# VinAIResearch/Counting-DETR

Measured on AMD Instinct MI355X. Metric: images/sec FSCD-147 2nd-stage train step, higher is better.
Workload: dtype forward bf16x3 (fp32 operands split hi+lo, 3 bf16 MFMAs per product); data / weight gradients bf16 (both operands rounded to bf16, 1 MFMA per product); fp32 accumulate, fp32 storage, fp32 attention softmax / norms / losses / optimizer; 1 GPU; FSCD-147 2nd-stage train step (ResNet-50-DC5 + RCDA enc6/dec6, Q=300 learned, 800x800, T=[37, 120]), fwd+matcher+loss+bwd+clip+AdamW; images_per_gpu=2, global_batch=2, parallelism=dp1, graph=True, precision=bf16x3, precision_backward=bf16, frozen_stage_prefetch=True

## Files before the change

### counting_detr_amd/csrc/api.hip

```cpp
#include <stdarg.h>
#include <stdio.h>

#include "../../include/cdetr_hip.h"
#include "common.h"

static thread_local char g_err[512] = "";

void cdetr_set_error(const char* fmt, ...) {
    va_list ap;
    va_start(ap, fmt);
    vsnprintf(g_err, sizeof(g_err), fmt, ap);
    va_end(ap);
}

extern "C" const char* cdetr_last_error(void) { return g_err; }
extern "C" int cdetr_abi_version(void) { return CDETR_ABI_VERSION; }

#include <stdlib.h>
#include <string.h>
extern char** environ;
namespace {
struct TuneEnvCheck {
    TuneEnvCheck() {
        if (getenv("CDETR_TUNING") != nullptr || environ == nullptr) return;
        static const char* const knobs[] = {"CDETR_DIRECT_MAX_BLOCKS", "CDETR_GEMM_DL", "CDETR_GEMM_FEWROW_SPLIT", "CDETR_GEMM_SPLITK", "CDETR_GEMM_VARIANT",
                                            "CDETR_LN_BWD_ROWS", "CDETR_LSAP_GENERIC", "CDETR_RCDA_HS", "CDETR_RCDA_PROBE", "CDETR_WGRAD_KP",
                                            "CDETR_WGRAD_VARIANT"};
        for (const char* k : knobs)
            if (getenv(k) != nullptr)
                fprintf(stderr, "libcdetr_hip: %s is set but CDETR_TUNING is not -- per-call tuning knobs are ignored without it\n", k);
    }
} g_tune_env_check;
}
```

### counting_detr_amd/csrc/matcher.hip

```cpp
#include "../../include/cdetr_hip.h"
#include "common.h"
#include <stdlib.h>

#pragma clang fp contract(off)

namespace {

__global__ __launch_bounds__(256) void match_cost_kernel(const float* __restrict__ logits, int ncls,
                                                         const float* __restrict__ boxes, const float* __restrict__ tgt,
                                                         const int* __restrict__ tgt_off, const int64_t* __restrict__ cost_off,
                                                         int Q, float w_class, float w_bbox, float w_giou,
                                                         float* __restrict__ cost) {
    const int b = blockIdx.y;
    const int t0 = tgt_off[b], T = tgt_off[b + 1] - t0;
    const long total = (long)Q * T;
    const bool transpose = T < Q;
    float* out = cost + cost_off[b];
    for (long idx = (long)blockIdx.x * 256 + threadIdx.x; idx < total; idx += (long)gridDim.x * 256) {
        int q, t;
        if (transpose) { t = (int)(idx / Q); q = (int)(idx - (long)t * Q); }
        else { q = (int)(idx / T); t = (int)(idx - (long)q * T); }
        const float x = logits[((long)b * Q + q) * ncls + 0];
        const float p = 1.f / (1.f + expf(-x));
        const float neg = (0.75f * (p * p)) * (-logf((1.f - p) + 1e-8f));
        const float pos = (0.25f * ((1.f - p) * (1.f - p))) * (-logf(p + 1e-8f));
        const float cost_class = pos - neg;
        const float* ob = boxes + ((long)b * Q + q) * 4;
        const float* tb = tgt + ((long)t0 + t) * 4;
        const float ocx = ob[0], ocy = ob[1], ow = ob[2], oh = ob[3];
        const float tcx = tb[0], tcy = tb[1], tw = tb[2], th = tb[3];
        const float cost_bbox = ((fabsf(ocx - tcx) + fabsf(ocy - tcy)) + fabsf(ow - tw)) + fabsf(oh - th);
        const float ox0 = ocx - 0.5f * ow, oy0 = ocy - 0.5f * oh, ox1 = ocx + 0.5f * ow, oy1 = ocy + 0.5f * oh;
        const float tx0 = tcx - 0.5f * tw, ty0 = tcy - 0.5f * th, tx1 = tcx + 0.5f * tw, ty1 = tcy + 0.5f * th;
        const float a1 = (ox1 - ox0) * (oy1 - oy0), a2 = (tx1 - tx0) * (ty1 - ty0);
        const float iw = fmaxf(fminf(ox1, tx1) - fmaxf(ox0, tx0), 0.f), ih = fmaxf(fminf(oy1, ty1) - fmaxf(oy0, ty0), 0.f);
        const float inter = iw * ih;
        const float uni = (a1 + a2) - inter;
        const float iou = inter / uni;
        const float ew = fmaxf(fmaxf(ox1, tx1) - fminf(ox0, tx0), 0.f), eh = fmaxf(fmaxf(oy1, ty1) - fminf(oy0, ty0), 0.f);
        const float area = ew * eh;
        const float giou = iou - (area - uni) / area;
        const float c = (w_bbox * cost_bbox + w_class * cost_class) + w_giou * (-giou);
        out[idx] = c;
    }
}

struct Cand {
    double val;
    int it;
    int unassigned;
};
__device__ __forceinline__ Cand better(const Cand& a, const Cand& b) {
    if (a.it < 0) return b;
    if (b.it < 0) return a;
    if (a.val < b.val) return a;
    if (b.val < a.val) return b;
    if (a.unassigned != b.unassigned) return a.unassigned ? a : b;
    if (a.unassigned) return (a.it > b.it) ? a : b;
    return (a.it < b.it) ? a : b;
}
__device__ __forceinline__ Cand shfl_xor_cand(const Cand& c, int m) {
    Cand r;
    r.val = __shfl_xor(c.val, m, 64);
    r.it = __shfl_xor(c.it, m, 64);
    r.unassigned = __shfl_xor(c.unassigned, m, 64);
    return r;
}

template <int NT>
__global__ __launch_bounds__(NT) void lsap_kernel(const float* __restrict__ cost_all, const int64_t* __restrict__ cost_off,
                                                  const int* __restrict__ tgt_off, int Q, int Mmax, int64_t* __restrict__ idx_i,
                                                  int64_t* __restrict__ idx_j, int* __restrict__ status, int nc_cap) {
    extern __shared__ __attribute__((aligned(16))) unsigned char lds[];
    __builtin_amdgcn_s_setprio(3);
    const int b = blockIdx.x;
    const int T = tgt_off[b + 1] - tgt_off[b];
    const bool transpose = T < Q;
    const int nr = transpose ? T : Q;
    const int nc = transpose ? Q : T;
    const float* cost = cost_all + cost_off[b];
    const int tid = threadIdx.x;
    int64_t* oi = idx_i + (long)b * Mmax;
    int64_t* oj = idx_j + (long)b * Mmax;
    for (int i = tid; i < Mmax; i += NT) { oi[i] = 0; oj[i] = 0; }
    __syncthreads();
    if (nr == 0) { if (tid == 0) status[b] = 0; return; }

    double* v = reinterpret_cast<double*>(lds);
    double* spc = v + nc_cap;
    double* u = spc + nc_cap;
    int* path = reinterpret_cast<int*>(u + nc_cap);
    int* row4col = path + nc_cap;
    int* remaining = row4col + nc_cap;
    int* col4row = remaining + nc_cap;
    unsigned char* SC = reinterpret_cast<unsigned char*>(col4row + nc_cap);
    unsigned char* SR = SC + nc_cap;
    __shared__ Cand wave_best[NT / 64];
    __shared__ int s_i, s_sink, s_num_remaining, s_bad;
    __shared__ double s_min;

    if (tid == 0) s_bad = 0;
    for (int j = tid; j < nc; j += NT) { v[j] = 0.0; path[j] = -1; row4col[j] = -1; }
    for (int i = tid; i < nr; i += NT) { u[i] = 0.0; col4row[i] = -1; }
    __syncthreads();
    {
        int bad = 0;
        for (long k = tid; k < (long)nr * nc; k += NT) {
            const float c = cost[k];
            if (c != c || c == -INFINITY) bad = 1;
        }
        if (bad) atomicOr(&s_bad, 1);
    }
    __syncthreads();
    if (s_bad) { if (tid == 0) status[b] = 2; return; }

    for (int cur = 0; cur < nr; ++cur) {
        for (int j = tid; j < nc; j += NT) { spc[j] = INFINITY; SC[j] = 0; remaining[j] = nc - j - 1; }
        for (int i = tid; i < nr; i += NT) SR[i] = 0;
        if (tid == 0) { s_i = cur; s_sink = -1; s_num_remaining = nc; s_min = 0.0; }
        __syncthreads();
        while (true) {
            const int i = s_i;
            const int num_remaining = s_num_remaining;
            const double min_val = s_min;
            const double ui = u[i];
            const float* crow = cost + (long)i * nc;
            Cand best;
            best.val = INFINITY; best.it = -1; best.unassigned = 0;
            for (int it = tid; it < num_remaining; it += NT) {
                const int j = remaining[it];
                const double r = ((min_val + (double)crow[j]) - ui) - v[j];
                double s = spc[j];
                if (r < s) { path[j] = i; spc[j] = r; s = r; }
                Cand c;
                c.val = s; c.it = it; c.unassigned = (row4col[j] == -1);
                best = better(best, c);
            }
#pragma unroll
            for (int m = 32; m > 0; m >>= 1) best = better(best, shfl_xor_cand(best, m));
            if (NT > 64) {
                if ((tid & 63) == 0) wave_best[tid >> 6] = best;
                __syncthreads();
                if (tid == 0) {
                    Cand bb = wave_best[0];
                    for (int wv = 1; wv < NT / 64; ++wv) bb = better(bb, wave_best[wv]);
                    wave_best[0] = bb;
                }
                __syncthreads();
                best = wave_best[0];
            }
            if (tid == 0) {
                SR[i] = 1;
                if (best.it < 0 || best.val == INFINITY) {
                    s_sink = -2;
                } else {
                    const int j = remaining[best.it];
                    s_min = best.val;
                    if (row4col[j] == -1) s_sink = j;
                    else s_i = row4col[j];
                    SC[j] = 1;
                    remaining[best.it] = remaining[num_remaining - 1];
                    s_num_remaining = num_remaining - 1;
                }
            }
            __syncthreads();
            if (s_sink != -1) break;
        }
        const int sink = s_sink;
        if (sink == -2) { if (tid == 0) status[b] = 1; return; }
        const double min_val = s_min;
        for (int i = tid; i < nr; i += NT) {
            if (i == cur) u[i] += min_val;
            else if (SR[i]) u[i] += min_val - spc[col4row[i]];
        }
        for (int j = tid; j < nc; j += NT)
            if (SC[j]) v[j] -= min_val - spc[j];
        __syncthreads();
        if (tid == 0) {
            int j = sink;
            while (true) {
                const int i = path[j];
                row4col[j] = i;
                const int t = col4row[i];
                col4row[i] = j;
                j = t;
                if (i == cur) break;
            }
        }
        __syncthreads();
    }
    if (!transpose) {
        for (int i = tid; i < nr; i += NT) { oi[i] = i; oj[i] = col4row[i]; }
    } else {
        for (int j = tid; j < nc; j += NT) remaining[j] = (row4col[j] != -1) ? 1 : 0;
        __syncthreads();
        if (tid == 0) {
            int run = 0;
            for (int j = 0; j < nc; ++j) { const int f = remaining[j]; remaining[j] = run; run += f; }
        }
        __syncthreads();
        for (int j = tid; j < nc; j += NT)
            if (row4col[j] != -1) { oi[remaining[j]] = j; oj[remaining[j]] = row4col[j]; }
    }
    if (tid == 0) status[b] = 0;
}


template <int CTRL, int ROW_MASK>
__device__ __forceinline__ double dpp_min_f64(double x) {
    const int lo = __double2loint(x), hi = __double2hiint(x);
    const int olo = __builtin_amdgcn_update_dpp(lo, lo, CTRL, ROW_MASK, 0xf, false);
    const int ohi = __builtin_amdgcn_update_dpp(hi, hi, CTRL, ROW_MASK, 0xf, false);
    const double o = __hiloint2double(ohi, olo);
    return (o < x) ? o : x;
}
template <int CTRL, int ROW_MASK>
__device__ __forceinline__ unsigned dpp_min_u32(unsigned x) {
    const unsigned o = (unsigned)__builtin_amdgcn_update_dpp((int)x, (int)x, CTRL, ROW_MASK, 0xf, false);
    return o < x ? o : x;
}
__device__ __forceinline__ void wave_lexmin(double& val, unsigned& key) {
    double m = val;
    m = dpp_min_f64<0xB1, 0xf>(m);
    m = dpp_min_f64<0x4E, 0xf>(m);
    m = dpp_min_f64<0x141, 0xf>(m);
    m = dpp_min_f64<0x140, 0xf>(m);
    m = dpp_min_f64<0x142, 0xa>(m);
    m = dpp_min_f64<0x143, 0xc>(m);
    const double gmin = __hiloint2double(__builtin_amdgcn_readlane(__double2hiint(m), 63), __builtin_amdgcn_readlane(__double2loint(m), 63));
    unsigned k = (val == gmin) ? key : 0xffffffffu;
    k = dpp_min_u32<0xB1, 0xf>(k);
    k = dpp_min_u32<0x4E, 0xf>(k);
    k = dpp_min_u32<0x141, 0xf>(k);
    k = dpp_min_u32<0x140, 0xf>(k);
    k = dpp_min_u32<0x142, 0xa>(k);
    k = dpp_min_u32<0x143, 0xc>(k);
    key = (unsigned)__builtin_amdgcn_readlane((int)k, 63);
    val = gmin;
}

template <int CPL, bool COST_LDS>
__global__ __launch_bounds__(64) void lsap_wave_kernel(const float* __restrict__ cost_all, const int64_t* __restrict__ cost_off,
                                                       const int* __restrict__ tgt_off, int Q, int Mmax,
                                                       int64_t* __restrict__ idx_i, int64_t* __restrict__ idx_j,
                                                       int* __restrict__ status) {
    extern __shared__ __attribute__((aligned(16))) unsigned char lds[];
    __builtin_amdgcn_s_setprio(3);
    const int b = blockIdx.x;
    const int T = tgt_off[b + 1] - tgt_off[b];
    const bool transpose = T < Q;
    const int nr = transpose ? T : Q;
    const int nc = transpose ? Q : T;
    const float* cost_g = cost_all + cost_off[b];
    const int lane = threadIdx.x;
    int64_t* oi = idx_i + (long)b * Mmax;
    int64_t* oj = idx_j + (long)b * Mmax;
    for (int i = lane; i < Mmax; i += 64) { oi[i] = 0; oj[i] = 0; }
    if (nr == 0) { if (lane == 0) status[b] = 0; return; }

    double* u = reinterpret_cast<double*>(lds);
    int* col4row = reinterpret_cast<int*>(u + nr);
    int* row4col = col4row + nr;
    int* remaining = row4col + nc;
    int* pathl = remaining + nc;
    float* cost_l = reinterpret_cast<float*>((reinterpret_cast<uintptr_t>(pathl + nc) + 15) & ~(uintptr_t)15);
    const float* cost = COST_LDS ? cost_l : cost_g;

    int bad = 0;
    const long ntot = (long)nr * nc;
    constexpr int LU = 16;
    if ((reinterpret_cast<uintptr_t>(cost_g) & 15) == 0) {
        const long n4 = ntot >> 2;
        const float4* g4 = reinterpret_cast<const float4*>(cost_g);
        for (long k0 = 0; k0 < n4; k0 += 64 * LU) {
            float4 t[LU];
#pragma unroll
            for (int q = 0; q < LU; ++q) t[q] = g4[min(k0 + lane + 64 * q, n4 - 1)];
#pragma unroll
            for (int q = 0; q < LU; ++q) {
                const long k = k0 + lane + 64 * q;
                if (k < n4) {
                    const float4 c = t[q];
                    if (c.x != c.x || c.x == -INFINITY || c.y != c.y || c.y == -INFINITY || c.z != c.z || c.z == -INFINITY ||
                        c.w != c.w || c.w == -INFINITY) bad = 1;
                    if (COST_LDS) *reinterpret_cast<float4*>(cost_l + 4 * k) = c;
                }
            }
        }
        for (long k = (n4 << 2) + lane; k < ntot; k += 64) {
            const float c = cost_g[k];
            if (c != c || c == -INFINITY) bad = 1;
            if (COST_LDS) cost_l[k] = c;
        }
    } else {
        for (long k0 = 0; k0 < ntot; k0 += 64 * LU) {
            float t[LU];
#pragma unroll
            for (int q = 0; q < LU; ++q) t[q] = cost_g[min(k0 + lane + 64 * q, ntot - 1)];
#pragma unroll
            for (int q = 0; q < LU; ++q) {
                const long k = k0 + lane + 64 * q;
                if (k < ntot) {
                    if (t[q] != t[q] || t[q] == -INFINITY) bad = 1;
                    if (COST_LDS) cost_l[k] = t[q];
                }
            }
        }
    }
    if (__any(bad)) { if (lane == 0) status[b] = 2; return; }
    for (int i = lane; i < nr; i += 64) { u[i] = 0.0; col4row[i] = -1; }
    for (int j = lane; j < nc; j += 64) row4col[j] = -1;

    double v[CPL], spc[CPL];
    int path[CPL], r4c[CPL];
    unsigned key[CPL];
    unsigned valid = 0;
#pragma unroll
    for (int c = 0; c < CPL; ++c) { v[c] = 0.0; path[c] = -1; r4c[c] = -1; if (lane + 64 * c < nc) valid |= 1u << c; }

    for (int cur = 0; cur < nr; ++cur) {
        {
            const float* crow0 = cost + (long)cur * nc;
            const double ui0 = u[cur];
            const double min0 = 0.0;
            double bval = INFINITY;
            unsigned bkey = 0xffffffffu;
            int best_c = 0;
#pragma unroll
            for (int c = 0; c < CPL; ++c) {
                const bool a = (valid >> c) & 1u;
                const int jj = a ? lane + 64 * c : 0;
                const double r = ((min0 + (double)crow0[jj]) - ui0) - v[c];
                const double s = (a & (r < INFINITY)) ? r : INFINITY;
                const unsigned p0 = (unsigned)(nc - 1 - (lane + 64 * c));
                const unsigned k = (r4c[c] == -1) ? (0x7fffffffu - p0) : (0x80000000u + p0);
                const bool better = a & ((s < bval) | ((s == bval) & (k < bkey)));
                bval = better ? s : bval;
                bkey = better ? k : bkey;
                best_c = better ? c : best_c;
            }
            const double my_val = bval;
            const unsigned my_key = bkey;
            wave_lexmin(bval, bkey);
            if (bkey != 0xffffffffu && bval != INFINITY && (bkey & 0x80000000u) == 0u) {
                const bool mine = (my_key == bkey) && (my_val == bval);
                const int wl = __builtin_ctzll(__ballot(mine));
                const int jstar = __builtin_amdgcn_readlane(lane + 64 * best_c, wl);
                if (lane == 0) {
                    u[cur] = ui0 + bval;
                    row4col[jstar] = cur;
                    col4row[cur] = jstar;
                }
#pragma unroll
                for (int c = 0; c < CPL; ++c) r4c[c] = (mine && best_c == c) ? cur : r4c[c];
                continue;
            }
        }
        unsigned sc = 0;
#pragma unroll
        for (int c = 0; c < CPL; ++c) {
            spc[c] = INFINITY;
            const unsigned p0 = (unsigned)(nc - 1 - (lane + 64 * c));
            key[c] = (r4c[c] == -1) ? (0x7fffffffu - p0) : (0x80000000u + p0);
        }
        for (int it = lane; it < nc; it += 64) remaining[it] = nc - 1 - it;
        int i = cur, num_remaining = nc, sink = -1;
        double min_val = 0.0;
        while (true) {
            const int last = num_remaining - 1;
            const int jlast = *reinterpret_cast<volatile int*>(remaining + last);
            const float* crow = cost + (long)i * nc;
            const double ui = u[i];
            double bval = INFINITY;
            unsigned bkey = 0xffffffffu;
            int best_c = 0;
            const unsigned act = valid & ~sc;
#pragma unroll
            for (int c = 0; c < CPL; ++c) {
                const bool a = (act >> c) & 1u;
                const int jj = ((valid >> c) & 1u) ? lane + 64 * c : 0;
                const double r = ((min_val + (double)crow[jj]) - ui) - v[c];
                const bool upd = a & (r < spc[c]);
                spc[c] = upd ? r : spc[c];
                path[c] = upd ? i : path[c];
                const bool better = a & ((spc[c] < bval) | ((spc[c] == bval) & (key[c] < bkey)));
                bval = better ? spc[c] : bval;
                bkey = better ? key[c] : bkey;
                best_c = better ? c : best_c;
            }
            const double my_val = bval;
            const unsigned my_key = bkey;
            wave_lexmin(bval, bkey);
            if (bkey == 0xffffffffu || bval == INFINITY) { sink = -2; break; }
            min_val = bval;
            const bool mine = (my_key == bkey) && (my_val == bval);
            const int wl = __builtin_ctzll(__ballot(mine));
            int my_r = r4c[0];
#pragma unroll
            for (int c = 1; c < CPL; ++c) my_r = (best_c == c) ? r4c[c] : my_r;
            const int jstar = __builtin_amdgcn_readlane(lane + 64 * best_c, wl);
            const int inext = __builtin_amdgcn_readlane(my_r, wl);
            const bool j_unassigned = (bkey & 0x80000000u) == 0u;
            const int best_it = j_unassigned ? (int)(0x7fffffffu - bkey) : (int)(bkey - 0x80000000u);
            sc |= mine ? (1u << best_c) : 0u;
            if (lane == 0) remaining[best_it] = jlast;
#pragma unroll
            for (int c = 0; c < CPL; ++c) {
                const unsigned nk = (r4c[c] == -1) ? (0x7fffffffu - (unsigned)best_it) : (0x80000000u + (unsigned)best_it);
                key[c] = (lane + 64 * c == jlast) ? nk : key[c];
            }
            num_remaining = last;
            if (j_unassigned) { sink = jstar; break; }
            i = inext;
        }
        if (sink == -2) { if (lane == 0) status[b] = 1; return; }
        if (lane == 0) u[cur] += min_val;
#pragma unroll
        for (int c = 0; c < CPL; ++c) {
            const int j = lane + 64 * c;
            if ((sc >> c) & 1u) {
                const double delta = min_val - spc[c];
                v[c] -= delta;
                if (j != sink) u[r4c[c]] += delta;
            }
            if (j < nc) pathl[j] = path[c];
        }
        if (lane == 0) {
            int j = sink;
            while (true) {
                const int ii = pathl[j];
                row4col[j] = ii;
                const int t = col4row[ii];
                col4row[ii] = j;
                j = t;
                if (ii == cur) break;
            }
        }
#pragma unroll
        for (int c = 0; c < CPL; ++c)
            if ((valid >> c) & 1u) r4c[c] = row4col[lane + 64 * c];
    }
    if (!transpose) {
        for (int i = lane; i < nr; i += 64) { oi[i] = i; oj[i] = col4row[i]; }
    } else {
        int base = 0;
        for (int j0 = 0; j0 < nc; j0 += 64) {
            const int j = j0 + lane;
            const int r = (j < nc) ? row4col[j] : -1;
            const unsigned long long m = __ballot(r != -1);
            if (r != -1) {
                const int rank = base + __popcll(m & ((1ull << lane) - 1ull));
                oi[rank] = j;
                oj[rank] = r;
            }
            base += __popcll(m);
        }
    }
    if (lane == 0) status[b] = 0;
}

struct WgSlot { double val; unsigned key; int jstar; int rnext; int pad_; };

template <int CPL>
__global__ __launch_bounds__(1024) void lsap_wg_kernel(const float* __restrict__ cost_all, const int64_t* __restrict__ cost_off,
                                                       const int* __restrict__ tgt_off, int Q, int Mmax, int64_t* __restrict__ idx_i,
                                                       int64_t* __restrict__ idx_j, int* __restrict__ status) {
    constexpr int NT = 1024, NW = 16;
    extern __shared__ __attribute__((aligned(16))) unsigned char lds[];
    __builtin_amdgcn_s_setprio(3);
    const int b = blockIdx.x;
    const int T = tgt_off[b + 1] - tgt_off[b];
    const bool transpose = T < Q;
    const int nr = transpose ? T : Q;
    const int nc = transpose ? Q : T;
    const float* __restrict__ cost = cost_all + cost_off[b];
    const int tid = threadIdx.x, lane = tid & 63, wv = tid >> 6;
    int64_t* oi = idx_i + (long)b * Mmax;
    int64_t* oj = idx_j + (long)b * Mmax;
    for (int i = tid; i < Mmax; i += NT) { oi[i] = 0; oj[i] = 0; }
    if (nr == 0) { if (tid == 0) status[b] = 0; return; }

    WgSlot* slots = reinterpret_cast<WgSlot*>(lds);
    double* u = reinterpret_cast<double*>(slots + 2 * NW);
    int* col4row = reinterpret_cast<int*>(u + nr);
    int* row4col = col4row + nr;
    int* remaining = row4col + nc;
    int* pathl = remaining + nc;
    __shared__ int s_bad;
    if (tid == 0) s_bad = 0;
    for (int i = tid; i < nr; i += NT) { u[i] = 0.0; col4row[i] = -1; }
    for (int j = tid; j < nc; j += NT) row4col[j] = -1;
    __syncthreads();
    {
        int bad = 0;
        const long ntot = (long)nr * nc;
        for (long k0 = 0; k0 < ntot; k0 += (long)NT * 8) {
            float t[8];
#pragma unroll
            for (int q = 0; q < 8; ++q) t[q] = cost[min(k0 + tid + (long)NT * q, ntot - 1)];
#pragma unroll
            for (int q = 0; q < 8; ++q) bad |= (t[q] != t[q] || t[q] == -INFINITY) ? 1 : 0;
        }
        if (bad) atomicOr(&s_bad, 1);
    }
    __syncthreads();
    if (s_bad) { if (tid == 0) status[b] = 2; return; }

    double v[CPL], spc[CPL];
    int path[CPL], r4c[CPL];
    unsigned key[CPL];
    unsigned valid = 0;
#pragma unroll
    for (int c = 0; c < CPL; ++c) { v[c] = 0.0; spc[c] = INFINITY; path[c] = -1; r4c[c] = -1; key[c] = 0xffffffffu; if (tid + NT * c < nc) valid |= 1u << c; }
    int parity = 0;

    auto wg_lexmin = [&](double& bval, unsigned& bkey, int best_c, int& jstar, int& rnext, bool& mine) __attribute__((always_inline)) {
        const double my_val = bval;
        const unsigned my_key = bkey;
        wave_lexmin(bval, bkey);
        const bool wmine = (my_key == bkey) && (my_val == bval) && (bkey != 0xffffffffu);
        const unsigned long long bal = __ballot(wmine);
        const int wl = bal ? __builtin_ctzll(bal) : 0;
        int my_r = r4c[0];
#pragma unroll
        for (int c = 1; c < CPL; ++c) my_r = (best_c == c) ? r4c[c] : my_r;
        const int wj = __builtin_amdgcn_readlane(tid + NT * best_c, wl);
        const int wr = __builtin_amdgcn_readlane(my_r, wl);
        WgSlot* sl = slots + parity * NW;
        if (lane == 0) { sl[wv].val = bval; sl[wv].key = bkey; sl[wv].jstar = wj; sl[wv].rnext = wr; }
        __syncthreads();
        double gv = sl[0].val;
        unsigned gk = sl[0].key;
        int gj = sl[0].jstar, gr = sl[0].rnext;
#pragma unroll
        for (int w2 = 1; w2 < NW; ++w2) {
            const double ov = sl[w2].val;
            const unsigned ok = sl[w2].key;
            const bool take = (ov < gv) | ((ov == gv) & (ok < gk));
            gv = take ? ov : gv;
            gk = take ? ok : gk;
            gj = take ? sl[w2].jstar : gj;
            gr = take ? sl[w2].rnext : gr;
        }
        parity ^= 1;
        mine = wmine && (my_key == gk) && (my_val == gv);
        bval = gv; bkey = gk; jstar = gj; rnext = gr;
    };

    for (int cur = 0; cur < nr; ++cur) {
        {
            const float* crow0 = cost + (long)cur * nc;
            const double ui0 = u[cur];
            double bval = INFINITY;
            unsigned bkey = 0xffffffffu;
            int best_c = 0;
            float cv[CPL];
#pragma unroll
            for (int c = 0; c < CPL; ++c) cv[c] = crow0[((valid >> c) & 1u) ? tid + NT * c : 0];
#pragma unroll
            for (int c = 0; c < CPL; ++c) {
                const bool a = (valid >> c) & 1u;
                const double r = ((0.0 + (double)cv[c]) - ui0) - v[c];
                const double s = (a & (r < INFINITY)) ? r : INFINITY;
                const unsigned p0 = (unsigned)(nc - 1 - (tid + NT * c));
                const unsigned k = (r4c[c] == -1) ? (0x7fffffffu - p0) : (0x80000000u + p0);
                const bool better = a & ((s < bval) | ((s == bval) & (k < bkey)));
                bval = better ? s : bval;
                bkey = better ? k : bkey;
                best_c = better ? c : best_c;
            }
            int jstar, rnext;
            bool mine;
            wg_lexmin(bval, bkey, best_c, jstar, rnext, mine);
            if (bkey != 0xffffffffu && bval != INFINITY && (bkey & 0x80000000u) == 0u) {
                if (tid == 0) {
                    u[cur] = ui0 + bval;
                    row4col[jstar] = cur;
                    col4row[cur] = jstar;
                }
#pragma unroll
                for (int c = 0; c < CPL; ++c) r4c[c] = (mine && best_c == c) ? cur : r4c[c];
                continue;
            }
        }
        unsigned sc = 0;
#pragma unroll
        for (int c = 0; c < CPL; ++c) {
            spc[c] = INFINITY;
            const unsigned p0 = (unsigned)(nc - 1 - (tid + NT * c));
            key[c] = (r4c[c] == -1) ? (0x7fffffffu - p0) : (0x80000000u + p0);
        }
        for (int it = tid; it < nc; it += NT) remaining[it] = nc - 1 - it;
        int i = cur, num_remaining = nc, sink = -1;
        double min_val = 0.0;
        while (true) {
            const int last = num_remaining - 1;
            const float* crow = cost + (long)i * nc;
            const double ui = u[i];
            double bval = INFINITY;
            unsigned bkey = 0xffffffffu;
            int best_c = 0;
            const unsigned act = valid & ~sc;
            float cv[CPL];
#pragma unroll
            for (int c = 0; c < CPL; ++c) cv[c] = crow[((valid >> c) & 1u) ? tid + NT * c : 0];
#pragma unroll
            for (int c = 0; c < CPL; ++c) {
                const bool a = (act >> c) & 1u;
                const double r = ((min_val + (double)cv[c]) - ui) - v[c];
                const bool upd = a & (r < spc[c]);
                spc[c] = upd ? r : spc[c];
                path[c] = upd ? i : path[c];
                const bool better = a & ((spc[c] < bval) | ((spc[c] == bval) & (key[c] < bkey)));
                bval = better ? spc[c] : bval;
                bkey = better ? key[c] : bkey;
                best_c = better ? c : best_c;
            }
            int jstar, inext;
            bool mine;
            wg_lexmin(bval, bkey, best_c, jstar, inext, mine);
            if (bkey == 0xffffffffu || bval == INFINITY) { sink = -2; break; }
            min_val = bval;
            const bool j_unassigned = (bkey & 0x80000000u) == 0u;
            const int best_it = j_unassigned ? (int)(0x7fffffffu - bkey) : (int)(bkey - 0x80000000u);
            sc |= mine ? (1u << best_c) : 0u;
            const int jlast = remaining[last];
            if (tid == 0) remaining[best_it] = jlast;
#pragma unroll
            for (int c = 0; c < CPL; ++c) {
                const unsigned nk = (r4c[c] == -1) ? (0x7fffffffu - (unsigned)best_it) : (0x80000000u + (unsigned)best_it);
                key[c] = (tid + NT * c == jlast) ? nk : key[c];
            }
            num_remaining = last;
            if (j_unassigned) { sink = jstar; break; }
            i = inext;
        }
        if (sink == -2) { if (tid == 0) status[b] = 1; return; }
        if (tid == 0) u[cur] += min_val;
#pragma unroll
        for (int c = 0; c < CPL; ++c) {
            const int j = tid + NT * c;
            if ((sc >> c) & 1u) {
                const double delta = min_val - spc[c];
                v[c] -= delta;
                if (j != sink) u[r4c[c]] += delta;
            }
            if (j < nc) pathl[j] = path[c];
        }
        __syncthreads();
        if (tid == 0) {
            int j = sink;
            while (true) {
                const int ii = pathl[j];
                row4col[j] = ii;
                const int t = col4row[ii];
                col4row[ii] = j;
                j = t;
                if (ii == cur) break;
            }
        }
        __syncthreads();
#pragma unroll
        for (int c = 0; c < CPL; ++c)
            if ((valid >> c) & 1u) r4c[c] = row4col[tid + NT * c];
    }
    __syncthreads();
    if (!transpose) {
        for (int i = tid; i < nr; i += NT) { oi[i] = i; oj[i] = col4row[i]; }
    } else {
        for (int j = tid; j < nc; j += NT) remaining[j] = (row4col[j] != -1) ? 1 : 0;
        __syncthreads();
        if (tid == 0) {
            int run = 0;
            for (int j = 0; j < nc; ++j) { const int f = remaining[j]; remaining[j] = run; run += f; }
        }
        __syncthreads();
        for (int j = tid; j < nc; j += NT)
            if (row4col[j] != -1) { oi[remaining[j]] = j; oj[remaining[j]] = row4col[j]; }
    }
    if (tid == 0) status[b] = 0;
}

inline size_t lds_bytes(int nc_cap) { return (size_t)nc_cap * (3 * 8 + 4 * 4 + 2) + 16; }
inline int round_cap(int nc) { return (nc + 15) & ~15; }

}

extern "C" int cdetr_match_cost(const float* logits, int32_t ncls, const float* boxes, const float* tgt,
                                const int32_t* tgt_off, const int64_t* cost_off, int32_t B, int32_t Q, float w_class,
                                float w_bbox, float w_giou, float* cost, void* stream) {
    CDETR_CHECK_ARG(logits && boxes && tgt_off && cost_off && cost && B > 0 && Q > 0 && ncls > 0, "cdetr_match_cost: bad args");
    dim3 grid(64, B);
    hipLaunchKernelGGL(match_cost_kernel, grid, dim3(256), 0, reinterpret_cast<hipStream_t>(stream), logits, ncls, boxes, tgt,
                       tgt_off, cost_off, Q, w_class, w_bbox, w_giou, cost);
    return cdetr_launch_status("cdetr_match_cost");
}

extern "C" int cdetr_lsap(const float* cost, const int64_t* cost_off, const int32_t* tgt_off, int32_t B, int32_t Q,
                          int32_t nc_max, int32_t Mmax, int64_t* idx_i, int64_t* idx_j, int32_t* status, void* stream) {
    CDETR_CHECK_ARG(cost && cost_off && tgt_off && idx_i && idx_j && status && B > 0 && Q > 0 && Mmax > 0 && nc_max >= Q,
                    "cdetr_lsap: bad args");
    const int cap = round_cap(nc_max);
    const size_t bytes = lds_bytes(cap);
    if (bytes > 158 * 1024) {
        cdetr_set_error("cdetr_lsap: max(Q, T) = %d exceeds the LDS-resident solver's capacity (3800)", nc_max);
        return CDETR_ERR_UNSUPPORTED;
    }
    hipStream_t st = reinterpret_cast<hipStream_t>(stream);
    if (nc_max <= 1024 && cdetr_tune_env("CDETR_LSAP_GENERIC") == nullptr) {
        const size_t state = (size_t)Mmax * 12 + (size_t)nc_max * 12 + 64;
        const size_t with_cost = state + (size_t)Mmax * nc_max * 4;
        const bool cost_lds = with_cost <= 156 * 1024;
        const size_t wb = cost_lds ? with_cost : state;
        auto go = [&](auto kern) {
            if (wb > 64 * 1024) (void)hipFuncSetAttribute(reinterpret_cast<const void*>(kern), hipFuncAttributeMaxDynamicSharedMemorySize, (int)wb);
            hipLaunchKernelGGL(kern, dim3(B), dim3(64), wb, st, cost, cost_off, tgt_off, Q, Mmax, idx_i, idx_j, status);
        };
        if (nc_max <= 128) { if (cost_lds) go(lsap_wave_kernel<2, true>); else go(lsap_wave_kernel<2, false>); }
        else if (nc_max <= 256) { if (cost_lds) go(lsap_wave_kernel<4, true>); else go(lsap_wave_kernel<4, false>); }
        else if (nc_max <= 320) { if (cost_lds) go(lsap_wave_kernel<5, true>); else go(lsap_wave_kernel<5, false>); }
        else if (nc_max <= 512) { if (cost_lds) go(lsap_wave_kernel<8, true>); else go(lsap_wave_kernel<8, false>); }
        else { if (cost_lds) go(lsap_wave_kernel<16, true>); else go(lsap_wave_kernel<16, false>); }
        return cdetr_launch_status("cdetr_lsap");
    }
    if (nc_max <= 1024) {
        if (bytes > 64 * 1024) (void)hipFuncSetAttribute(reinterpret_cast<const void*>(lsap_kernel<64>), hipFuncAttributeMaxDynamicSharedMemorySize, (int)bytes);
        hipLaunchKernelGGL(lsap_kernel<64>, dim3(B), dim3(64), bytes, st, cost, cost_off, tgt_off, Q, Mmax, idx_i, idx_j, status, cap);
    } else if (nc_max <= 4096 && cdetr_tune_env("CDETR_LSAP_GENERIC") == nullptr) {
        const size_t wb = 2 * 16 * sizeof(WgSlot) + (size_t)Mmax * 12 + (size_t)nc_max * 12 + 64;
        if (wb > 64 * 1024) {
            const void* fn = nc_max <= 2048 ? reinterpret_cast<const void*>(lsap_wg_kernel<2>) : reinterpret_cast<const void*>(lsap_wg_kernel<4>);
            if (hipFuncSetAttribute(fn, hipFuncAttributeMaxDynamicSharedMemorySize, (int)wb) != hipSuccess) {
                (void)hipGetLastError();
                cdetr_set_error("cdetr_lsap: %zu bytes of LDS for %d x %d problems exceed the device limit", wb, Mmax, nc_max);
                return CDETR_ERR_UNSUPPORTED;
            }
        }
        if (nc_max <= 2048) hipLaunchKernelGGL(lsap_wg_kernel<2>, dim3(B), dim3(1024), wb, st, cost, cost_off, tgt_off, Q, Mmax, idx_i, idx_j, status);
        else hipLaunchKernelGGL(lsap_wg_kernel<4>, dim3(B), dim3(1024), wb, st, cost, cost_off, tgt_off, Q, Mmax, idx_i, idx_j, status);
    } else {
        if (bytes > 64 * 1024) (void)hipFuncSetAttribute(reinterpret_cast<const void*>(lsap_kernel<256>), hipFuncAttributeMaxDynamicSharedMemorySize, (int)bytes);
        hipLaunchKernelGGL(lsap_kernel<256>, dim3(B), dim3(256), bytes, st, cost, cost_off, tgt_off, Q, Mmax, idx_i, idx_j, status, cap);
    }
    return cdetr_launch_status("cdetr_lsap");
}
```

Before: 240.6 images/s.

## Speed up wave LSAP solver with 4-wave cost staging and ballot-based lexmin

The Hungarian matcher kernel now launches 256 threads so four waves share the cost-matrix copy into LDS and the NaN check; only wave 0 then runs the serial augmentation. The wave arg-min uses a ballot to skip the second key reduction when a single lane holds the minimum, and per-lane candidate selection becomes a tree merge. The first row's greedy step is folded into the augmenting search. A compile-time timing probe and tuning env knobs are added; the change is small relative to the whole train step.

Result: no change. 241.0 images/s, median of 3 (+0.2%).

```diff
diff --git a/counting_detr_amd/csrc/api.hip b/counting_detr_amd/csrc/api.hip
--- a/counting_detr_amd/csrc/api.hip
+++ b/counting_detr_amd/csrc/api.hip
@@ -24,7 +24,7 @@
     TuneEnvCheck() {
         if (getenv("CDETR_TUNING") != nullptr || environ == nullptr) return;
         static const char* const knobs[] = {"CDETR_DIRECT_MAX_BLOCKS", "CDETR_GEMM_DL", "CDETR_GEMM_FEWROW_SPLIT", "CDETR_GEMM_SPLITK", "CDETR_GEMM_VARIANT",
-                                            "CDETR_LN_BWD_ROWS", "CDETR_LSAP_GENERIC", "CDETR_RCDA_HS", "CDETR_RCDA_PROBE", "CDETR_WGRAD_KP",
+                                            "CDETR_LN_BWD_ROWS", "CDETR_LSAP_GENERIC", "CDETR_LSAP_LOAD1", "CDETR_LSAP_PROBE", "CDETR_RCDA_HS", "CDETR_RCDA_PROBE", "CDETR_WGRAD_KP",
                                             "CDETR_WGRAD_VARIANT"};
         for (const char* k : knobs)
             if (getenv(k) != nullptr)
diff --git a/counting_detr_amd/csrc/matcher.hip b/counting_detr_amd/csrc/matcher.hip
--- a/counting_detr_amd/csrc/matcher.hip
+++ b/counting_detr_amd/csrc/matcher.hip
@@ -219,28 +219,44 @@
     const unsigned o = (unsigned)__builtin_amdgcn_update_dpp((int)x, (int)x, CTRL, ROW_MASK, 0xf, false);
     return o < x ? o : x;
 }
-__device__ __forceinline__ void wave_lexmin(double& val, unsigned& key) {
-    double m = val;
+__device__ __forceinline__ double wave_min_f64(double m) {
     m = dpp_min_f64<0xB1, 0xf>(m);
     m = dpp_min_f64<0x4E, 0xf>(m);
     m = dpp_min_f64<0x141, 0xf>(m);
     m = dpp_min_f64<0x140, 0xf>(m);
     m = dpp_min_f64<0x142, 0xa>(m);
     m = dpp_min_f64<0x143, 0xc>(m);
-    const double gmin = __hiloint2double(__builtin_amdgcn_readlane(__double2hiint(m), 63), __builtin_amdgcn_readlane(__double2loint(m), 63));
-    unsigned k = (val == gmin) ? key : 0xffffffffu;
+    return __hiloint2double(__builtin_amdgcn_readlane(__double2hiint(m), 63), __builtin_amdgcn_readlane(__double2loint(m), 63));
+}
+__device__ __forceinline__ unsigned wave_min_u32(unsigned k) {
     k = dpp_min_u32<0xB1, 0xf>(k);
     k = dpp_min_u32<0x4E, 0xf>(k);
     k = dpp_min_u32<0x141, 0xf>(k);
     k = dpp_min_u32<0x140, 0xf>(k);
     k = dpp_min_u32<0x142, 0xa>(k);
     k = dpp_min_u32<0x143, 0xc>(k);
-    key = (unsigned)__builtin_amdgcn_readlane((int)k, 63);
+    return (unsigned)__builtin_amdgcn_readlane((int)k, 63);
+}
+__device__ __forceinline__ int wave_lexmin(double& val, unsigned& key) {
+    const double gmin = wave_min_f64(val);
+    const unsigned long long holders = __ballot(val == gmin);
+    int wl;
+    if (__builtin_popcountll(holders) == 1) {
+        wl = __builtin_ctzll(holders);
+        key = (unsigned)__builtin_amdgcn_readlane((int)key, wl);
+    } else {
+        const unsigned mk = (val == gmin) ? key : 0xffffffffu;
+        const unsigned kmin = wave_min_u32(mk);
+        const unsigned long long own = __ballot(mk == kmin);
+        wl = own ? __builtin_ctzll(own) : 0;
+        key = kmin;
+    }
     val = gmin;
-}
-
-template <int CPL, bool COST_LDS>
-__global__ __launch_bounds__(64) void lsap_wave_kernel(const float* __restrict__ cost_all, const int64_t* __restrict__ cost_off,
+    return wl;
+}
+
+template <int CPL, bool COST_LDS, bool PROBE = false>
+__global__ __launch_bounds__(256) void lsap_wave_kernel(const float* __restrict__ cost_all, const int64_t* __restrict__ cost_off,
                                                        const int* __restrict__ tgt_off, int Q, int Mmax,
                                                        int64_t* __restrict__ idx_i, int64_t* __restrict__ idx_j,
                                                        int* __restrict__ status) {
@@ -252,19 +268,27 @@
     const int nr = transpose ? T : Q;
     const int nc = transpose ? Q : T;
     const float* cost_g = cost_all + cost_off[b];
-    const int lane = threadIdx.x;
+    const int tid = threadIdx.x, NT = blockDim.x;
+    const int lane = tid & 63, wave = __builtin_amdgcn_readfirstlane(tid >> 6);
     int64_t* oi = idx_i + (long)b * Mmax;
     int64_t* oj = idx_j + (long)b * Mmax;
-    for (int i = lane; i < Mmax; i += 64) { oi[i] = 0; oj[i] = 0; }
-    if (nr == 0) { if (lane == 0) status[b] = 0; return; }
+    if (wave == 0) for (int i = lane; i < Mmax; i += 64) { oi[i] = 0; oj[i] = 0; }
+    if (nr == 0) { if (tid == 0) status[b] = 0; return; }
+    unsigned long long pr[16] = {};
+    auto now = [&]() __attribute__((always_inline)) -> unsigned long long {
+        if constexpr (PROBE) { const unsigned long long t = __builtin_amdgcn_s_memtime(); asm volatile("s_waitcnt lgkmcnt(0)" ::: "memory"); return t; }
+        return 0ull;
+    };
+    pr[0] = now();
 
     double* u = reinterpret_cast<double*>(lds);
     int* col4row = reinterpret_cast<int*>(u + nr);
     int* row4col = col4row + nr;
     int* remaining = row4col + nc;
     int* pathl = remaining + nc;
-    float* cost_l = reinterpret_cast<float*>((reinterpret_cast<uintptr_t>(pathl + nc) + 15) & ~(uintptr_t)15);
-    const float* cost = COST_LDS ? cost_l : cost_g;
+    float* cost_l = reinterpret_cast<float*>(lds + (((unsigned)(nr + nc) * 12u + 15u) & ~15u));
+    const float* cost;
+    if constexpr (COST_LDS) cost = cost_l; else cost = cost_g;
 
     int bad = 0;
     const long ntot = (long)nr * nc;
@@ -272,13 +296,13 @@
     if ((reinterpret_cast<uintptr_t>(cost_g) & 15) == 0) {
         const long n4 = ntot >> 2;
         const float4* g4 = reinterpret_cast<const float4*>(cost_g);
-        for (long k0 = 0; k0 < n4; k0 += 64 * LU) {
+        for (long k0 = 0; k0 < n4; k0 += (long)NT * LU) {
             float4 t[LU];
 #pragma unroll
-            for (int q = 0; q < LU; ++q) t[q] = g4[min(k0 + lane + 64 * q, n4 - 1)];
+            for (int q = 0; q < LU; ++q) t[q] = g4[min(k0 + tid + (long)NT * q, n4 - 1)];
 #pragma unroll
             for (int q = 0; q < LU; ++q) {
-                const long k = k0 + lane + 64 * q;
+                const long k = k0 + tid + (long)NT * q;
                 if (k < n4) {
                     const float4 c = t[q];
                     if (c.x != c.x || c.x == -INFINITY || c.y != c.y || c.y == -INFINITY || c.z != c.z || c.z == -INFINITY ||
@@ -287,19 +311,19 @@
                 }
             }
         }
-        for (long k = (n4 << 2) + lane; k < ntot; k += 64) {
+        for (long k = (n4 << 2) + tid; k < ntot; k += NT) {
             const float c = cost_g[k];
             if (c != c || c == -INFINITY) bad = 1;
             if (COST_LDS) cost_l[k] = c;
         }
     } else {
-        for (long k0 = 0; k0 < ntot; k0 += 64 * LU) {
+        for (long k0 = 0; k0 < ntot; k0 += (long)NT * LU) {
             float t[LU];
 #pragma unroll
-            for (int q = 0; q < LU; ++q) t[q] = cost_g[min(k0 + lane + 64 * q, ntot - 1)];
+            for (int q = 0; q < LU; ++q) t[q] = cost_g[min(k0 + tid + (long)NT * q, ntot - 1)];
 #pragma unroll
             for (int q = 0; q < LU; ++q) {
-                const long k = k0 + lane + 64 * q;
+                const long k = k0 + tid + (long)NT * q;
                 if (k < ntot) {
                     if (t[q] != t[q] || t[q] == -INFINITY) bad = 1;
                     if (COST_LDS) cost_l[k] = t[q];
@@ -307,9 +331,19 @@
             }
         }
     }
-    if (__any(bad)) { if (lane == 0) status[b] = 2; return; }
+    __shared__ int s_bad[4];
+    {
+        const int wbad = __any(bad) ? 1 : 0;
+        if (lane == 0) s_bad[wave] = wbad;
+    }
+    __syncthreads();
+    if (wave != 0) return;
+    bad = s_bad[0];
+    for (int w = 1; w < (NT >> 6); ++w) bad |= s_bad[w];
+    if (bad) { if (lane == 0) status[b] = 2; return; }
     for (int i = lane; i < nr; i += 64) { u[i] = 0.0; col4row[i] = -1; }
     for (int j = lane; j < nc; j += 64) row4col[j] = -1;
+    pr[1] = now();
 
     double v[CPL], spc[CPL];
     int path[CPL], r4c[CPL];
@@ -318,33 +352,64 @@
 #pragma unroll
     for (int c = 0; c < CPL; ++c) { v[c] = 0.0; path[c] = -1; r4c[c] = -1; if (lane + 64 * c < nc) valid |= 1u << c; }
 
+    [[maybe_unused]] unsigned long long trow = pr[1];
+    struct Pick { double v; unsigned k; int c; };
+    auto merge = [](const Pick& x, const Pick& y, bool ya) __attribute__((always_inline)) -> Pick {
+        const bool take = ya & ((y.v < x.v) | ((y.v == x.v) & (y.k < x.k)));
+        Pick r;
+        r.v = take ? y.v : x.v; r.k = take ? y.k : x.k; r.c = take ? y.c : x.c;
+        return r;
+    };
+    auto lane_best = [&](const double* val, const unsigned* ky, unsigned act) __attribute__((always_inline)) -> Pick {
+        constexpr int NN = (CPL + 1) / 2;
+        Pick n[NN];
+#pragma unroll
+        for (int c = 0; c < CPL; c += 2) {
+            const bool a0 = (act >> c) & 1u;
+            Pick x;
+            x.v = a0 ? val[c] : INFINITY; x.k = a0 ? ky[c] : 0xffffffffu; x.c = c;
+            if (c + 1 < CPL) {
+                Pick y;
+                y.v = val[c + 1]; y.k = ky[c + 1]; y.c = c + 1;
+                x = merge(x, y, (act >> (c + 1)) & 1u);
+            }
+            n[c / 2] = x;
+        }
+#pragma unroll
+        for (int s = 1; s < NN; s *= 2)
+#pragma unroll
+            for (int k = 0; k + s < NN; k += 2 * s) n[k] = merge(n[k], n[k + s], true);
+        return n[0];
+    };
     for (int cur = 0; cur < nr; ++cur) {
+        unsigned sc = 0;
+        int i = cur, num_remaining = nc, sink = -1;
+        double min_val = 0.0;
+        [[maybe_unused]] unsigned long long ta = 0;
         {
             const float* crow0 = cost + (long)cur * nc;
             const double ui0 = u[cur];
-            const double min0 = 0.0;
-            double bval = INFINITY;
-            unsigned bkey = 0xffffffffu;
-            int best_c = 0;
+            float cf[CPL];
+#pragma unroll
+            for (int c = 0; c < CPL; ++c) cf[c] = crow0[((valid >> c) & 1u) ? lane + 64 * c : 0];
 #pragma unroll
             for (int c = 0; c < CPL; ++c) {
-                const bool a = (valid >> c) & 1u;
-                const int jj = a ? lane + 64 * c : 0;
-                const double r = ((min0 + (double)crow0[jj]) - ui0) - v[c];
-                const double s = (a & (r < INFINITY)) ? r : INFINITY;
+                const double r = ((min_val + (double)cf[c]) - ui0) - v[c];
+                spc[c] = (((valid >> c) & 1u) & (r < INFINITY)) ? r : INFINITY;
                 const unsigned p0 = (unsigned)(nc - 1 - (lane + 64 * c));
-                const unsigned k = (r4c[c] == -1) ? (0x7fffffffu - p0) : (0x80000000u + p0);
-                const bool better = a & ((s < bval) | ((s == bval) & (k < bkey)));
-                bval = better ? s : bval;
-                bkey = better ? k : bkey;
-                best_c = better ? c : best_c;
-            }
-            const double my_val = bval;
-            const unsigned my_key = bkey;
-            wave_lexmin(bval, bkey);
-            if (bkey != 0xffffffffu && bval != INFINITY && (bkey & 0x80000000u) == 0u) {
-                const bool mine = (my_key == bkey) && (my_val == bval);
-                const int wl = __builtin_ctzll(__ballot(mine));
+                key[c] = (r4c[c] == -1) ? (0x7fffffffu - p0) : (0x80000000u + p0);
+            }
+            const Pick best = lane_best(spc, key, valid);
+            double bval = best.v;
+            unsigned bkey = best.k;
+            const int best_c = best.c;
+            [[maybe_unused]] const double my_val = bval;
+            [[maybe_unused]] const unsigned long long tr0 = now();
+            const int wl = wave_lexmin(bval, bkey);
+            if constexpr (PROBE) pr[12] += __builtin_popcountll(__ballot(my_val == bval)) != 1;
+            if (bkey == 0xffffffffu || bval == INFINITY) { if (lane == 0) status[b] = 1; return; }
+            if ((bkey & 0x80000000u) == 0u) {
+                const bool mine = lane == wl;
                 const int jstar = __builtin_amdgcn_readlane(lane + 64 * best_c, wl);
                 if (lane == 0) {
                     u[cur] = ui0 + bval;
@@ -353,48 +418,58 @@
                 }
 #pragma unroll
                 for (int c = 0; c < CPL; ++c) r4c[c] = (mine && best_c == c) ? cur : r4c[c];
+                if constexpr (PROBE) { const unsigned long long t = now(); pr[3] += 1; pr[4] += t - trow; pr[13] += t - tr0; trow = t; }
                 continue;
             }
-        }
-        unsigned sc = 0;
-#pragma unroll
-        for (int c = 0; c < CPL; ++c) {
-            spc[c] = INFINITY;
-            const unsigned p0 = (unsigned)(nc - 1 - (lane + 64 * c));
-            key[c] = (r4c[c] == -1) ? (0x7fffffffu - p0) : (0x80000000u + p0);
-        }
-        for (int it = lane; it < nc; it += 64) remaining[it] = nc - 1 - it;
-        int i = cur, num_remaining = nc, sink = -1;
-        double min_val = 0.0;
+#pragma unroll
+            for (int c = 0; c < CPL; ++c) path[c] = (spc[c] < INFINITY) ? cur : path[c];
+            for (int it = lane; it < nc; it += 64) remaining[it] = nc - 1 - it;
+            {
+                int my_r = r4c[0];
+#pragma unroll
+                for (int c = 1; c < CPL; ++c) my_r = (best_c == c) ? r4c[c] : my_r;
+                i = __builtin_amdgcn_readlane(my_r, wl);
+                const int best_it = (int)(bkey - 0x80000000u);
+                sc = (lane == wl) ? (1u << best_c) : 0u;
+                if (lane == 0) remaining[best_it] = 0;
+                const unsigned nk = (r4c[0] == -1) ? (0x7fffffffu - (unsigned)best_it) : (0x80000000u + (unsigned)best_it);
+                key[0] = (lane == 0) ? nk : key[0];
+            }
+            num_remaining = nc - 1;
+            min_val = bval;
+            if constexpr (PROBE) { asm volatile("" : "+v"(key[0]), "+v"(key[CPL - 1])); ta = now(); pr[5] += 1; pr[6] += ta - trow; }
+        }
         while (true) {
             const int last = num_remaining - 1;
-            const int jlast = *reinterpret_cast<volatile int*>(remaining + last);
+            const int jlast = remaining[last];
             const float* crow = cost + (long)i * nc;
             const double ui = u[i];
-            double bval = INFINITY;
-            unsigned bkey = 0xffffffffu;
-            int best_c = 0;
             const unsigned act = valid & ~sc;
+            float cf[CPL];
+            double r[CPL];
+#pragma unroll
+            for (int c = 0; c < CPL; ++c) cf[c] = crow[((valid >> c) & 1u) ? lane + 64 * c : 0];
+#pragma unroll
+            for (int c = 0; c < CPL; ++c) r[c] = ((min_val + (double)cf[c]) - ui) - v[c];
 #pragma unroll
             for (int c = 0; c < CPL; ++c) {
-                const bool a = (act >> c) & 1u;
-                const int jj = ((valid >> c) & 1u) ? lane + 64 * c : 0;
-                const double r = ((min_val + (double)crow[jj]) - ui) - v[c];
-                const bool upd = a & (r < spc[c]);
-                spc[c] = upd ? r : spc[c];
+                const bool upd = ((act >> c) & 1u) & (r[c] < spc[c]);
+                spc[c] = upd ? r[c] : spc[c];
                 path[c] = upd ? i : path[c];
-                const bool better = a & ((spc[c] < bval) | ((spc[c] == bval) & (key[c] < bkey)));
-                bval = better ? spc[c] : bval;
-                bkey = better ? key[c] : bkey;
-                best_c = better ? c : best_c;
-            }
-            const double my_val = bval;
-            const unsigned my_key = bkey;
-            wave_lexmin(bval, bkey);
+            }
+            const Pick best = lane_best(spc, key, act);
+            double bval = best.v;
+            unsigned bkey = best.k;
+            const int best_c = best.c;
+            [[maybe_unused]] const double my_val = bval;
+            [[maybe_unused]] unsigned long long tb = 0, tc = 0;
+            if constexpr (PROBE) { asm volatile("" : "+v"(bkey)); tb = now(); }
+            const int wl = wave_lexmin(bval, bkey);
+            if constexpr (PROBE) { asm volatile("" : "+s"(bkey)); tc = now(); pr[7] += 1; pr[8] += tb - ta; pr[9] += tc - tb; }
             if (bkey == 0xffffffffu || bval == INFINITY) { sink = -2; break; }
+            if constexpr (PROBE) pr[12] += __builtin_popcountll(__ballot(my_val == bval)) != 1;
             min_val = bval;
-            const bool mine = (my_key == bkey) && (my_val == bval);
-            const int wl = __builtin_ctzll(__ballot(mine));
+            const bool mine = lane == wl;
             int my_r = r4c[0];
 #pragma unroll
             for (int c = 1; c < CPL; ++c) my_r = (best_c == c) ? r4c[c] : my_r;
@@ -410,6 +485,7 @@
                 key[c] = (lane + 64 * c == jlast) ? nk : key[c];
             }
             num_remaining = last;
+            if constexpr (PROBE) { asm volatile("" : "+v"(key[0]), "+v"(key[CPL - 1])); ta = now(); pr[10] += ta - tc; }
             if (j_unassigned) { sink = jstar; break; }
             i = inext;
         }
@@ -439,6 +515,7 @@
 #pragma unroll
         for (int c = 0; c < CPL; ++c)
             if ((valid >> c) & 1u) r4c[c] = row4col[lane + 64 * c];
+        if constexpr (PROBE) { asm volatile("" : "+v"(r4c[0]), "+v"(r4c[CPL - 1])); const unsigned long long t = now(); pr[11] += t - ta; trow = t; }
     }
     if (!transpose) {
         for (int i = lane; i < nr; i += 64) { oi[i] = i; oj[i] = col4row[i]; }
@@ -457,6 +534,12 @@
         }
     }
     if (lane == 0) status[b] = 0;
+    if constexpr (PROBE) {
+        pr[2] = now();
+        unsigned long long* ps = reinterpret_cast<unsigned long long*>(idx_i + (long)gridDim.x * Mmax) + (long)b * 16;
+        if (lane == 0)
+            for (int k = 0; k < 16; ++k) ps[k] = pr[k];
+    }
 }
 
 struct WgSlot { double val; unsigned key; int jstar; int rnext; int pad_; };
@@ -517,10 +600,8 @@
     auto wg_lexmin = [&](double& bval, unsigned& bkey, int best_c, int& jstar, int& rnext, bool& mine) __attribute__((always_inline)) {
         const double my_val = bval;
         const unsigned my_key = bkey;
-        wave_lexmin(bval, bkey);
-        const bool wmine = (my_key == bkey) && (my_val == bval) && (bkey != 0xffffffffu);
-        const unsigned long long bal = __ballot(wmine);
-        const int wl = bal ? __builtin_ctzll(bal) : 0;
+        const int wl = wave_lexmin(bval, bkey);
+        const bool wmine = (lane == wl) && (bkey != 0xffffffffu);
         int my_r = r4c[0];
 #pragma unroll
         for (int c = 1; c < CPL; ++c) my_r = (best_c == c) ? r4c[c] : my_r;
@@ -712,10 +793,16 @@
         const size_t with_cost = state + (size_t)Mmax * nc_max * 4;
         const bool cost_lds = with_cost <= 156 * 1024;
         const size_t wb = cost_lds ? with_cost : state;
+        const int nt = cdetr_tune_env("CDETR_LSAP_LOAD1") != nullptr ? 64 : 256;
         auto go = [&](auto kern) {
             if (wb > 64 * 1024) (void)hipFuncSetAttribute(reinterpret_cast<const void*>(kern), hipFuncAttributeMaxDynamicSharedMemorySize, (int)wb);
-            hipLaunchKernelGGL(kern, dim3(B), dim3(64), wb, st, cost, cost_off, tgt_off, Q, Mmax, idx_i, idx_j, status);
+            hipLaunchKernelGGL(kern, dim3(B), dim3(nt), wb, st, cost, cost_off, tgt_off, Q, Mmax, idx_i, idx_j, status);
         };
+        if (cdetr_tune_env("CDETR_LSAP_PROBE") != nullptr) {
+            if (!(cost_lds && nc_max > 256 && nc_max <= 320)) { cdetr_set_error("cdetr_lsap: the phase probe is built for 256 < max(Q, T) <= 320 with the costs in LDS"); return CDETR_ERR_ARG; }
+            go(lsap_wave_kernel<5, true, true>);
+            return cdetr_launch_status("cdetr_lsap(probe)");
+        }
         if (nc_max <= 128) { if (cost_lds) go(lsap_wave_kernel<2, true>); else go(lsap_wave_kernel<2, false>); }
         else if (nc_max <= 256) { if (cost_lds) go(lsap_wave_kernel<4, true>); else go(lsap_wave_kernel<4, false>); }
         else if (nc_max <= 320) { if (cost_lds) go(lsap_wave_kernel<5, true>); else go(lsap_wave_kernel<5, false>); }
```
